# patrickltobing/cyclevae-vc

Measured on AMD Instinct MI355X. Metric: mcep_frames_per_sec_hu1024_ld32_cyc2, higher is better.
Workload: dtype f32 (every matrix product on exact fp32 operands: each operand carried as three fp16 limbs x = l0 + l1/2^11 + l2/2^22, six v_mfma_f32_32x32x16_f16 per product, f32 accumulate; dropped terms < 2^-33 of a product; gates, carried state, projection and outputs f32)

## Files before the change

cyclevae-vc_amd/csrc/cvae_exact3.h:

```cpp
#pragma once
#include <cvae_intrin.h>

#if defined(__HIP_DEVICE_COMPILE__)
#define CVAE_V6_IN_AGPR(x) asm volatile("" : "+a"(x))
#else
#define CVAE_V6_IN_AGPR(x) ((void)0)
#endif

struct Step6Params {
    const float* gx0;
    const float* w2s;
    float* hbuf;
    long mtot;
    float* hx;
    const float* wrec3;
    const float* afold3;
    const float* cfold;
    const float* bhn;
    const float* xt;
    int Tp, Cp;
    int B, Bp, H, T;
    unsigned* flags;
    int* status;
    long long* prof;
    const float* wyT;
    const float* dy;
    int Co;
    int rts;
    int want_f32;
    int exp;
    int backoff;
    const float* gx;
    long gx_bstride;
};

__global__ void k_prep_wrec3(const float* wrec2, float* wrec3, int H, int KPW, int* unfit) {
    const int nch = H >> 4, NB = H >> 3;
    const long idx = (long)blockIdx.x * blockDim.x + threadIdx.x;
    if (idx < (long)NB * 4 * KPW * 512) {
        const int e = (int)(idx & 7), lane = (int)((idx >> 3) & 63);
        const int s = (int)((idx >> 9) % KPW), wave = (int)(((idx >> 9) / KPW) & 3), c = (int)((idx >> 9) / KPW / 4);
        const int col = lane & 31, kh = lane >> 5, g = col >> 3, u = col & 7, j = 8 * c + u;
        const int k = 16 * (wave * KPW + s) + 8 * kh + e;
        float w = 0.0f;
        if (k < H) w = wrec2[((((long)(j >> 4) * 4 + g) * nch + (k >> 4)) * 16 + (j & 15)) * 16 + (k & 15)];
        unsigned short l0, l1, l2;
        cvae_split3_f16(w, l0, l1, l2);
        cvae_flag_unfit(unfit, w);
        unsigned short* dst = (unsigned short*)wrec3 + ((((long)c * 4 + wave) * KPW + s) * 3) * 512 + lane * 8 + e;
        dst[0] = l0;
        dst[512] = l1;
        dst[1024] = l2;
    }
}

__global__ void k_prep_wrec3_l2b(const float* wrec2, unsigned char* w2s, int H, int KPW) {
    const int nch = H >> 4, NB = H >> 3;
    const long idx = (long)blockIdx.x * blockDim.x + threadIdx.x;
    if (idx < (long)NB * 4 * KPW * 512) {
        const int e = (int)(idx & 7), lane = (int)((idx >> 3) & 63);
        const int s = (int)((idx >> 9) % KPW), wave = (int)(((idx >> 9) / KPW) & 3), c = (int)((idx >> 9) / KPW / 4);
        const int col = lane & 31, kh = lane >> 5, g = col >> 3, u = col & 7, j = 8 * c + u;
        const int k = 16 * (wave * KPW + s) + 8 * kh + e;
        float w = 0.0f;
        if (k < H) w = wrec2[((((long)(j >> 4) * 4 + g) * nch + (k >> 4)) * 16 + (j & 15)) * 16 + (k & 15)];
        unsigned short l0, l1;
        unsigned char l2;
        cvae_split3_f16b8(w, l0, l1, l2);
        w2s[idx] = l2;
    }
}

__global__ void k_prep_afold3l(const float* afold, float* afold3, int H, int Kfe, int KFW, int* unfit) {
    const int NB = H >> 3;
    const long idx = (long)blockIdx.x * blockDim.x + threadIdx.x;
    if (idx < (long)NB * 4 * KFW * 512) {
        const int e = (int)(idx & 7), lane = (int)((idx >> 3) & 63);
        const int s = (int)((idx >> 9) % KFW), wave = (int)(((idx >> 9) / KFW) & 3), c = (int)((idx >> 9) / KFW / 4);
        const int col = lane & 31, kh = lane >> 5, g = col >> 3, u = col & 7;
        const int k = 16 * (wave * KFW + s) + 8 * kh + e;
        const float w = (g < 3 && k < Kfe) ? afold[(long)(g * H + 8 * c + u) * Kfe + k] : 0.0f;
        unsigned short l0, l1, l2;
        cvae_split3_f16(w, l0, l1, l2);
        cvae_flag_unfit(unfit, w);
// ... 61 lines not shown
            CVAE_V6_IN_AGPR(w0[s]);
            CVAE_V6_IN_AGPR(w1[s]);
            CVAE_V6_IN_AGPR(w2[s]);
        }
    }
    {
        const float* src = p.afold3 + ((long)c * 4 + wave) * (KFW * 3 * 256);
        float* dst = wfl + wave * (KFW * LIMBS * 256);
#pragma unroll
        for (int s = 0; s < KFW; ++s)
#pragma unroll
            for (int m = 0; m < LIMBS; ++m)
                *(f32x4*)(dst + (s * LIMBS + m) * 256 + lane * 4) = *(const f32x4*)(src + (s * 3 + m) * 256 + lane * 4);
    }
    __syncthreads();
    const float* wfw = wfl + wave * (KFW * LIMBS * 256) + lane * 4;
    const float bhn = p.bhn[j];
    const float cf0 = HOIST ? 0.f : p.cfold[j], cf1 = HOIST ? 0.f : p.cfold[H + j], cf2 = HOIST ? 0.f : p.cfold[2 * H + j];
    const int ntile = ti < nrt ? (nrt - ti + rts - 1) / rts : 0, ntask = p.T * ntile;
    long long pc[PROF ? 4 : 1] = {};
    f32x4 x4[2 * RF];
    f32x2 x2[RF];
    const unsigned char* xw = nullptr;
    auto set_x = [&](int k) {
        const int tt = k / ntile, ii = ti + (k % ntile) * rts;
        xw = (const unsigned char*)p.xt + (((long)ii * p.Tp + tt) * (p.Cp >> 3) + 2 * (wave * KFW) + kh) * 1280;
    };
    auto load_x = [&](int s) {
        x4[2 * (s % RF)] = *(const f32x4*)(xw + s * 2560 + lc * 16);
        x4[2 * (s % RF) + 1] = *(const f32x4*)(xw + s * 2560 + 512 + lc * 16);
        if constexpr (LIMBS == 3) x2[s % RF] = *(const f32x2*)(xw + s * 2560 + 1024 + lc * 8);
    };
    float gq0 = 0.f, gq1 = 0.f, gq2 = 0.f;
    auto load_g = [&](int k) {
        const int tt = k / ntile, gr = (ti + (k % ntile) * rts) * 32 + row;
        if (gr < p.B) {
            const float* g = p.gx + (long)gr * p.gx_bstride + (long)tt * 3 * H + j;
            gq0 = g[0]; gq1 = g[H]; gq2 = g[2 * H];
        }
    };
    constexpr bool FPRE = CVAE_V6_FPRE && !HOIST && LIMBS == 3 && !W2S && KPW <= 16;
    constexpr bool FW0_EARLY = KFW <= 6;
    f32x4 fw[FPRE ? 2 * LIMBS : 1];
    auto load_fw = [&](int s) {
#pragma unroll
        for (int m = 0; m < LIMBS; ++m) fw[(s & 1) * LIMBS + m] = *(const f32x4*)(wfw + (s * LIMBS + m) * 256);
    };
    auto fw_op = [&](int s, int m) -> f32x4 {
        if constexpr (FPRE) return fw[(s & 1) * LIMBS + m];
        else return *(const f32x4*)(wfw + (s * LIMBS + m) * 256);
    };
    float hkeep0 = 0.f, hkeep1 = 0.f;
    const int backoff = (p.exp >> 8) ? (p.exp >> 8) - 1 : p.backoff;
    if constexpr (HOIST) {
        if (ntask > 0) load_g(0);
    } else if (ntask > 0) {
        set_x(0);
#pragma unroll
        for (int s = 0; s < RF; ++s) load_x(s);
    }
    if constexpr (FPRE && FW0_EARLY) { if (ntask > 0) load_fw(0); }
    unsigned fpre = 0u;
    for (int k = 0; k < ntask; ++k) {
        long long c0 = 0;
        if constexpr (PROF) c0 = cvae_clock();
        const int t = k / ntile, i = ti + (k % ntile) * rts;
        const unsigned row0 = (unsigned)(t * p.Bp + i * 32), tile0 = row0 >> 5;
        f32x16 a0 = cvae_zero16(), a1 = cvae_zero16(), a2 = cvae_zero16(), a3 = cvae_zero16();
        if constexpr (FPRE && !FW0_EARLY) load_fw(0);
#pragma unroll
        for (int s = 0; s < KFW; ++s) {
            const f32x4 l0 = x4[2 * (s % RF)], l1 = x4[2 * (s % RF) + 1];
            if constexpr (FPRE) {
                if (s + 1 < KFW) load_fw(s + 1);
                cvae_sched_fence();
            }
            const f32x4 b0 = fw_op(s, 0);
            const f32x4 b1 = fw_op(s, 1);
            a0 = cvae_mfma_32x32x16_f16(l0, b0, a0);
            a1 = cvae_mfma_32x32x16_f16(l0, b1, a1);
            if constexpr (LIMBS == 3) {
                const f32x4 l2 = cvae_bf8x8_to_h8(x2[s % RF]);
                const f32x4 b2 = fw_op(s, 2);
                a2 = cvae_mfma_32x32x16_f16(l1, b1, a2);
                if constexpr (W2S) a2 = cvae_mfma_32x32x16_f16(l0, b2, a2);
                else a3 = cvae_mfma_32x32x16_f16(l0, b2, a3);
                a1 = cvae_mfma_32x32x16_f16(l1, b0, a1);
                a2 = cvae_mfma_32x32x16_f16(l2, b0, a2);
            } else {
                a2 = cvae_mfma_32x32x16_f16(l1, b0, a2);
            }
            cvae_sched_fence();
            if (s + RF < KFW) load_x(s + RF);
        }
        if constexpr (PROF) { const long long c1 = cvae_clock(); pc[0] += c1 - c0; c0 = c1; }
        const bool pre_ok = ntile > 1 && k > 0 && cvae_wave_all(fpre >= (unsigned)t);
        if (t > 0 && !pre_ok) {
            unsigned spins = 0;
            if (ntile == 1)
                for (int q = 0; q < backoff; ++q) cvae_sleep_64();
            for (;;) {
                unsigned f = (unsigned)t;
                if (lane < 2 * KPW && 2 * s_lo + lane < NB) f = cvae_atomic_load_agent(p.flags + (long)i * NB + 2 * s_lo + lane);
                if (cvae_wave_all(f >= (unsigned)t)) break;
                cvae_sleep();
                if (++spins > (1u << 22)) {
                    p.status[0] = 2;
                    break;
                }
            }
        }
        cvae_compiler_fence();
        if constexpr (PROF) { const long long c1 = cvae_clock(); pc[1] += c1 - c0; c0 = c1; }
        const int grow = i * 32 + row;
        const bool live = grow < p.B;
        const bool keep1 = ntile == 2 && (k & 1);
        float gxr = HOIST ? gq0 : cf0, gxz = HOIST ? gq1 : cf1, gxn = HOIST ? gq2 : cf2, hold = keep1 ? hkeep1 : hkeep0;
        auto gate_inputs = [&]() {
            if (live) {
                if (t == 0 && p.gx0) {
                    const float* g0p = p.gx0 + (long)grow * 3 * H + j;
                    gxr += g0p[0]; gxz += g0p[H]; gxn += g0p[2 * H];
                } else if (t == 0 && p.dy) cvae_t0_fix(p.wyT, p.dy, p.Co, H, j, grow, gxr, gxz, gxn);
                if (t == 0) {
                    hold = cvae_buf_load_f1_sc1(hb, (unsigned)(row * 64 + (j & 15) * 4), ((unsigned)(j >> 4) * mtot + row0) * 64u);
                } else if (ntile > 2) {
                    const unsigned so = ((unsigned)(j >> 4) * tstride + tile0) * 2560u, okh = (unsigned)((j >> 3) & 1);
                    const unsigned vo = okh * 512u + (unsigned)(row * 16 + (u >> 1) * 4);
                    const int sh = (u & 1) * 16;
                    const unsigned q0 = __builtin_bit_cast(unsigned, cvae_buf_load_f1_sc1(xb_, vo, so));
                    const unsigned q1 = __builtin_bit_cast(unsigned, cvae_buf_load_f1_sc1(xb_, vo, so + 1024u));
                    float third = 0.0f;
                    if constexpr (LIMBS == 3) {
                        const unsigned q2 = __builtin_bit_cast(unsigned, cvae_buf_load_f1_sc1(xb_, 2048u + okh * 256u + (unsigned)(row * 8 + (u >> 2) * 4), so));
                        third = cvae_bf8_to_f32((unsigned char)(q2 >> ((u & 3) * 8))) * (S1 / CVAE_L2_SCALE);
                    }
                    hold = cvae_f16_bits_to_f32((unsigned short)(q0 >> sh)) + (cvae_f16_bits_to_f32((unsigned short)(q1 >> sh)) + third) * S1;
                }
            }
        };
        if constexpr (KPW >= 32) gate_inputs();
        f32x4 hc[2 * RD];
        f32x2 hb2[RD];
        const unsigned tsel = (p.exp & 1) ? (unsigned)i : tile0;
        auto load_h = [&](int s) {
            const unsigned so = ((unsigned)(s_lo + s) * tstride + tsel) * 2560u;
            hc[2 * (s % RD)] = cvae_buf_load_f4(xb_, voff, so);
            hc[2 * (s % RD) + 1] = cvae_buf_load_f4(xb_, voff, so + 1024u);
            if constexpr (LIMBS == 3) hb2[s % RD] = cvae_buf_load_f2(xb_, voff2, so);
        };
        f32x2 w2r[W2S ? RW : 1];
        const float* w2base = W2S ? p.w2s + ((long)c * 4 + wave) * KPW * 128 + lane * 2 : nullptr;
        auto load_w2 = [&](int s) { w2r[s % RW] = *(const f32x2*)(w2base + s * 128); };
        if constexpr (W2S) {
#pragma unroll
            for (int s = 0; s < RW; ++s) load_w2(s);
        }
#pragma unroll
        for (int s = 0; s < RD; ++s) load_h(s);
        if constexpr (KPW < 32) gate_inputs();
#pragma unroll
        for (int s = 0; s < KPW; ++s) {
            const f32x4 l0 = hc[2 * (s % RD)], l1 = hc[2 * (s % RD) + 1];
// ... 11 lines not shown
            }
            cvae_sched_fence();
            if (s + RD < KPW) load_h(s + RD);
            if constexpr (W2S) { if (s + RW < KPW) load_w2(s + RW); }
        }
        cvae_sched_fence();
        const int xmode = HOIST ? 0 : (p.exp >> 5) & 3;
        if constexpr (HOIST) {
            if (k + 1 < ntask) load_g(k + 1);
        } else {
            if (k + 1 < ntask) set_x(k + 1);
            if (k + 1 < ntask && (xmode == 0 || (xmode == 2 && wave != 0))) {
#pragma unroll
                for (int s = 0; s < RF; ++s) load_x(s);
            }
        }
#pragma unroll
        for (int q = 0; q < 16; ++q)
            red[(wave * 32 + (q & 3) + 8 * (q >> 2) + 4 * kh) * RS + lc] =
                LIMBS == 3 ? a0[q] + (a1[q] + (a2[q] + a3[q]) * S1) * S1 : a0[q] + (a1[q] + a2[q]) * S1;
        if constexpr (PROF) { const long long c1 = cvae_clock(); pc[2] += c1 - c0; c0 = c1; }
        __syncthreads();
        {
            float hn_ = 0.0f;
            if (live) {
                float sg[4];
#pragma unroll
                for (int g = 0; g < 4; ++g)
                    sg[g] = red[(0 * 32 + row) * RS + g * 8 + u] + red[(1 * 32 + row) * RS + g * 8 + u] +
                            red[(2 * 32 + row) * RS + g * 8 + u] + red[(3 * 32 + row) * RS + g * 8 + u];
                const float rg = cvae_sigmoid_fast(gxr + sg[0]);
                const float zg = cvae_sigmoid_fast(gxz + sg[1]);
                const float ng = cvae_tanh_fast(gxn + sg[2] + rg * (sg[3] + bhn));
                hn_ = ng + zg * (hold - ng);
            }
            if (keep1) hkeep1 = hn_; else hkeep0 = hn_;
            hsh[row * 8 + u] = hn_;
            unsigned short l0, l1;
            unsigned char l2;
            cvae_split3_f16b8(hn_, l0, l1, l2);
            hl[row * 8 + u] = l0;
            hl[256 + row * 8 + u] = l1;
            ((unsigned char*)(hl + 512))[row * 8 + u] = l2;
        }
        __syncthreads();
        if (tid < 64) {
            const unsigned so = ((unsigned)(c >> 1) * tstride + tile0 + (unsigned)(p.Bp >> 5)) * 2560u;
            cvae_buf_store_f4_sc1(xb_, (unsigned)(c & 1) * 512u + (unsigned)(tid & 31) * 16u, so + (unsigned)(tid >> 5) * 1024u,
                                  *(const f32x4*)(hl + tid * 8));
            if (LIMBS == 3 && tid < 32)
                cvae_buf_store_f2_sc1(xb_, 2048u + (unsigned)(c & 1) * 256u + (unsigned)tid * 8u, so, *(const f32x2*)(hl + 512 + tid * 4));
            cvae_drain_vmem();
            cvae_wave_barrier();
            if (tid == 0) cvae_atomic_store_agent(p.flags + (long)i * NB + c, (unsigned)(t + 1));
        } else if (tid < 128 && p.want_f32) {
            const int l = tid - 64, r = l >> 1, half = l & 1;
            *(f32x4*)(p.hbuf + (((long)(c >> 1) * p.mtot + row0 + p.Bp + r) * 16 + (c & 1) * 8 + half * 4)) =
                *(const f32x4*)(hsh + r * 8 + half * 4);
        }
        if constexpr (!HOIST) {
            if (k + 1 < ntask && (xmode == 1 || (xmode == 2 && wave == 0))) {
#pragma unroll
                for (int s = 0; s < RF; ++s) load_x(s);
            }
        }
        if (ntile > 1 && k + 1 < ntask) {
            const int kn = k + 1, tn = kn / ntile, in_ = ti + (kn % ntile) * rts;
            fpre = (unsigned)tn;
            if (tn > 0 && lane < 2 * KPW && 2 * s_lo + lane < NB)
                fpre = cvae_atomic_load_agent(p.flags + (long)in_ * NB + 2 * s_lo + lane);
        }
        if constexpr (FPRE && FW0_EARLY) { if (k + 1 < ntask) load_fw(0); }
        if constexpr (PROF) { const long long c1 = cvae_clock(); pc[3] += c1 - c0; c0 = c1; }
    }
    if constexpr (PROF) {
        if (p.prof && tid == 64 * ((p.exp >> 2) & 3))
            for (int q = 0; q < 4; ++q) p.prof[(long)blockIdx.x * 4 + q] = pc[q];
    }
}

struct Out6Params {
    const float* hx;
    long mtot;
    const float* wo3;
    const float* bo2;
    int H, Bp, T, B, ncell, Co, clamp_from;
    float clamp_min;
    float* out[CVAE_MAX_CELLS];
};

__global__ void k_prep_wo3(const float* wo2, float* wo3, int H, int Cop, int NT, int* unfit) {
    const int nk = H >> 4;
    const long idx = (long)blockIdx.x * blockDim.x + threadIdx.x;
    if (idx < (long)NT * nk * 512) {
        const int e = (int)(idx & 7), lane = (int)((idx >> 3) & 63), s = (int)((idx >> 9) % nk), n = (int)((idx >> 9) / nk);
        const int col = 32 * n + (lane & 31), k = 16 * s + 8 * (lane >> 5) + e;
        const float w = col < Cop ? wo2[(long)col * H + k] : 0.0f;
        unsigned short l0, l1, l2;
        cvae_split3_f16(w, l0, l1, l2);
        cvae_flag_unfit(unfit, w);
        unsigned short* dst = (unsigned short*)wo3 + (((long)n * nk + s) * 3) * 512 + lane * 8 + e;
        dst[0] = l0;
        dst[512] = l1;
        dst[1024] = l2;
    }
}

template <int KPW>
__global__ __launch_bounds__(256) void k_outproj_v6(Out6Params p) {
    constexpr float S1 = 1.0f / 2048.0f;
    constexpr int RS = 36;
    const int tid = threadIdx.x, wave = cvae_uniform(tid >> 6), lane = tid & 63, lc = lane & 31, kh = lane >> 5;
    const int nk = p.H >> 4, nt32 = p.Bp >> 5;
    const int n = blockIdx.y;
    const long tile = (long)nt32 + blockIdx.x;
    float* red = (float*)CVAE_SMEM;
    const long tstride = p.mtot >> 5;
    f32x16 a0 = cvae_zero16(), a1 = cvae_zero16(), a2 = cvae_zero16(), a3 = cvae_zero16();
    constexpr int RD = KPW < 4 ? KPW : 4;
    f32x4 ha[2 * RD], wb[3 * RD];
    f32x2 hb[RD];
    auto load = [&](int s) {
        const int sg = wave * KPW + s;
// ... 90 lines not shown
```

cyclevae-vc_amd/csrc/cvae_lib.hip:

```cpp
#include <cvae_intrin.h>

#include <stdarg.h>
#include <stdio.h>
#include <stdlib.h>
#include <string.h>

#include <atomic>
#include <map>
#include <mutex>
#include <new>
#include <utility>
#include <vector>

#include "cvae_kernels.h"
#include "cvae_train_kernels.h"
#include "cvae_deep.h"
#include "cyclevae_hip.h"

namespace {

thread_local char g_err[512] = "";

enum OptId {
    OPT_V6_LIMBS_H64, OPT_NO_LL, OPT_MAX_RT, OPT_LL_BACKOFF, OPT_EXP, OPT_GEMM_FORCE, OPT_GEMM_LOG, OPT_TRAIN_OLD_GEMM,
    OPT_GEMM_TRACE, OPT_TRAIN_PER_STEP, OPT_TRAIN_PROF, OPT_TRAIN_BACKOFF, OPT_TRAIN_FP32_MFMA, OPT_TRAIN_BWD_PER_STEP, OPT_TRAIN_KERNEL, OPT_X3_TILE, OPT_BWD_OVERFLOW_AT, OPT_GEMM_MAX_SPLIT, OPT_BWD_KS, OPT_COOP_LAUNCH, OPT_V6_LIMBS_H2048, OPT_V6_W2S_H64, OPT_STEP_COL_TILES, OPT_TRAIN_PROFILE, OPT_TRAIN_XMAP, OPT_MASKS_ON_SIDE, OPT_V6_BACKOFF, OPT_TRAIN_BWD_BACKOFF, OPT_LL_ROW_PAD, OPT_GEMM_MIN_DEPTH, OPT_TRAIN_BWD_GEOM, OPT_BWD_W3_L1_H64, OPT_TRAIN_FWD_GEOM, OPT_TRAIN_FWD_BACKOFF, OPT_EXACT_RANGE_AT, OPT_DTW_BATCH_COST, OPT_COUNT
};
struct OptEntry { const char* name; long dflt; };
const OptEntry g_opt[OPT_COUNT] = {
    {"v6_limbs_h64", 3},
    {"no_ll", 0},
    {"max_rt", 0},
    {"ll_backoff", -1},
    {"exp", 0},
    {"gemm_force", 0},
    {"gemm_log", 0},
    {"train_old_gemm", 0},
    {"gemm_trace", 0},
    {"train_per_step", 0},
    {"train_prof", 0},
    {"train_backoff", 32},
    {"train_fp32_mfma", 0},
    {"train_bwd_per_step", 0},
    {"train_kernel", 0},
    {"x3_tile", 0},
    {"bwd_overflow_at", 60000},
    {"gemm_max_split", 16},
    {"bwd_ks", 8},
    {"coop_launch", 0},
    {"v6_limbs_h2048", 3},
    {"v6_w2s_h64", 0},
    {"step_col_tiles", 0},
    {"train_profile", 0},
    {"train_xmap", 0},
    {"masks_on_side", 1},
    {"v6_backoff", -1},
    {"train_bwd_backoff", -1},
    {"ll_row_pad", 0},
    {"gemm_min_depth", 128},
    {"train_bwd_geom", -1},
    {"bwd_w3_l1_h64", 0},
    {"train_fwd_geom", -1},
    {"train_fwd_backoff", -1},
    {"exact_range_at", 65504},
    {"dtw_batch_cost", 1},
};

struct ProfEvents {
    std::vector<hipEvent_t> start, stop;
    std::vector<int> rows, cin;
    size_t used = 0;
};
enum { TPROF_FWD = 0, TPROF_BWD = 1, TPROF_GEMM = 2, TPROF_WGRAD = 3, TPROF_CLASSES = 4 };
struct TrainProfEvents {
    std::vector<hipEvent_t> start, stop;
    std::vector<int> cls;
    std::vector<double> flop;
    size_t used = 0;
};
struct SideDone { const void* scratch; hipEvent_t ev; };

}

struct cvae_ctx {
    int32_t* status_sink = nullptr;
    long draw_row0 = 0, draw_rows = 0, draw_frames = 0, draw_parts = 1;
    long opt[OPT_COUNT];
    ProfEvents prof;
    TrainProfEvents tprof;
    hipStream_t side = nullptr;
    SideDone side_done[8] = {};
    hipEvent_t side_ready = nullptr, side_join = nullptr, side_last = nullptr;
    int side_cap = 0;
    hipEvent_t mask_fork = nullptr, mask_join = nullptr;
    unsigned side_evict = 0;
    int32_t* gemm_ran = nullptr;
    std::map<const void*, std::pair<int, unsigned long>> train_var;
    unsigned long train_var_tick = 0;
    std::map<const void*, bool> image_unfit;
    int range_serial = 0;
    std::atomic<unsigned> ll_train_launch{1u};
};

namespace {

thread_local cvae_ctx* tl_ctx = nullptr;
inline cvae_ctx& cx() { return *tl_ctx; }
inline long opt(OptId i) { return tl_ctx->opt[i]; }
struct CtxScope {
    cvae_ctx* prev;
    explicit CtxScope(cvae_ctx* c) : prev(tl_ctx) {
        tl_ctx = c;
        g_cvae_coop_launch = (int)c->opt[OPT_COOP_LAUNCH];
    }
    ~CtxScope() { tl_ctx = prev; }
};

int fail(int code, const char* fmt, ...) {
// ... 129 lines not shown
}
inline bool exact3_fused(const Dims& m) { return find_v6(m) != nullptr; }
inline bool exact3_ok(const Dims& m) { return exact3_fused(m) || find_v6h(m) != nullptr; }
inline int v6_limbs(const Dims& m) {
    return (m.H == 64 && opt(OPT_V6_LIMBS_H64) == 2) || (m.H == 2048 && opt(OPT_V6_LIMBS_H2048) == 2) ? 2 : 3;
}
inline bool v6_w2s(const Dims& m) { return v6_limbs(m) == 3 && (m.H == 2048 || (m.H == 64 && opt(OPT_V6_W2S_H64))); }

struct Prep {
    long afold, afold3, afold_h, afold_t, cfold, wrec, wrec2, wrec_h, wrec_t, wrec_l2b, bhn, wyT, wo, bo, wo2, bo2, wo3, sin_w, sin_b, sout_w,
        sout_b, range, total;
};

Prep prep_layout(const Dims& m, bool sin, bool sout) {
    Prep p;
    long o = 0;
    auto take = [&](long n) { long r = o; o += up(n, 64); return r; };
    p.afold = take((long)m.H3 * m.Kfe);
    p.afold3 = take((long)m.nch * 4 * m.KFW * 3 * 256);
    p.afold_h = take((long)m.nch * 4 * ((m.KFW + 1) / 2) * 6 * 256);
    p.cfold = take(m.H3);
    p.wrec = take((long)(m.H / 4) * m.nch * 256);
    p.wrec2 = take((long)m.nch * 4 * m.nch * 256);
    p.wrec_h = take((long)m.nch * 4 * (m.H / 32) * 2 * 256);
    p.wrec_t = exact3_ok(m) ? take((long)(m.H / 8) * 4 * exact3_kpw(m) * 3 * 256) : -1;
    p.afold_t = exact3_fused(m) ? take((long)(m.H / 8) * 4 * m.KFW * 3 * 256) : -1;
    p.wrec_l2b = exact3_ok(m) ? take((long)(m.H / 8) * 4 * exact3_kpw(m) * 128) : -1;
    p.bhn = take(m.H);
    p.wyT = take((long)m.H3 * m.Co);
    p.wo = take((long)m.Cop * m.H);
    p.bo = take(m.Cop);
    p.wo2 = take((long)m.Cop * m.H);
    p.bo2 = take(m.Cop);
    p.wo3 = exact3_ok(m) ? take((long)((m.Cop + 31) / 32) * (m.H / 16) * 3 * 256) : -1;
    p.sin_w = sin ? take((long)m.C * m.C) : -1;
    p.sin_b = sin ? take(m.C) : -1;
    p.sout_w = sout ? take((long)m.Co * m.Co) : -1;
    p.sout_b = sout ? take(m.Co) : -1;
    p.range = take(64);
    p.total = o;
    return p;
}

struct Work {
    long status, xnp, xs, xs_plane, xt, xt_slack, gx, hbuf, hs, y, dy, gx0, prof, flags, total;
    int Bp, Tp, prof_blocks;
    long mtot;
};

inline int eval_row_pad(const Dims& m, int Brows) {
    return Brows <= 3 ? 16 : (exact3_ok(m) || Brows > 16 ? (int)up(Brows, 32) : 16);
}

Work work_layout(const Dims& m, int Brows, int T) {
    Work w;
    w.Bp = eval_row_pad(m, Brows);
    w.Tp = T + 2 * m.pad;
    w.mtot = (long)(T + 1) * w.Bp;
    long o = 0;
    auto take = [&](long n) { long r = o; o += up(n, 64); return r; };
    w.status = take(64);
    w.xnp = take((long)Brows * w.Tp * m.Cp + 64L * m.KFW + 64);
    w.xs_plane = up((long)Brows * w.Tp * m.Cp + 64L * m.KFW + 64, 8);
    w.xs = take(w.xs_plane);
    w.xt_slack = (64L * m.KFW / 8 + 2) * 640 + 64;
    w.xt = exact3_fused(m) && w.Bp % 32 == 0 ? take(((long)w.Bp * w.Tp * m.Cp * 5 / 2 + w.xt_slack) / 2 + 8) : -1;
    w.gx = take((long)Brows * w.Tp * m.H3);
    w.hbuf = take((long)m.nch * w.mtot * 16);
    w.hs = take((long)m.nch * w.mtot * 24);
    w.y = take((long)T * w.Bp * m.Cop);
    w.dy = take((long)w.Bp * m.Co);
    w.gx0 = take((long)w.Bp * m.H3);
    w.prof_blocks = 256;
    w.prof = take(w.prof_blocks * 8L);
    w.flags = take((long)(w.Bp / 16) * m.nch);
    w.total = o;
    return w;
}

inline int row_tiles_per_block(int cus, int per_tile, int ntiles) {
    int rts = per_tile > 0 ? cus / per_tile : 1;
    rts = rts < 1 ? 1 : (rts > ntiles ? ntiles : rts);
    if (opt(OPT_MAX_RT) >= 1 && opt(OPT_MAX_RT) < rts) rts = (int)opt(OPT_MAX_RT);
    return rts;
}

struct PassFacts {
    bool h_in, y_last, h_last, many_draws;
};
enum { PRO_ROWS = 0, PRO_DRAWS = 1, PRO_TILES = 2 };
enum { PROJ_GEMM = 0, PROJ_FUSED = 1, PROJ_V6 = 2 };
struct EvalPlan {
    int form;
    void (*k6)(Step6Params);
    void (*k5)(Step3Params);
    void (*k4)(Step3Params);
    void (*kout6)(Out6Params);
    int rts;
    int backoff;
    bool limbs;
    bool pairs;
    bool gx0_ready;
    bool want_f32;
    int prologue, proj;
};

inline int plain_projection(const Dims& m, bool y_last) {
    const int ntn = m.Cop / 16;
    return !y_last && (ntn == 1 || ntn == 4 || ntn == 8) ? PROJ_FUSED : PROJ_GEMM;
}

inline bool generic_resident(const Dims& m, int cus) { return cus <= 0 || m.H / 4 <= cus; }

EvalPlan plan_eval_pass(const Dims& m, int Brows, int T, int flags, int cus, bool unfit, const PassFacts& f) {
    EvalPlan pn;
    memset(&pn, 0, sizeof(pn));
    if (unfit) flags &= ~CVAE_FLAG_SPLIT_F16;
    const int Bp = eval_row_pad(m, Brows);
    const long mtot = (long)(T + 1) * Bp;
    const bool persistent = (flags & CVAE_FLAG_PERSISTENT) && T > 1, generic = (flags & CVAE_FLAG_GENERIC_STEP) != 0;
    const bool hoisted = (flags & CVAE_FLAG_HOISTED_FRONTEND) != 0, exact = persistent && (flags & CVAE_FLAG_EXACT3) && !generic;
    const V6Inst* i6 = find_v6(m, v6_limbs(m), v6_w2s(m));
    const V6Inst* i6h = find_v6h(m, v6_limbs(m), v6_w2s(m));
    const Fused16Inst* i16 = find_fused16(m);
    if (exact && Brows <= 3 && T < 65536 && m.H % 64 == 0 && m.H <= 1024 && cus >= m.H / 4 && !opt(OPT_NO_LL)) {
        pn.form = CVAE_EVAL_LL;
        pn.backoff = opt(OPT_LL_BACKOFF) >= 0 ? (int)opt(OPT_LL_BACKOFF) : (Brows == 1 ? 22 : 20);
    } else if (exact && !unfit && !hoisted && i6 && Bp % 32 == 0 && cus >= m.H / 8 && (long)m.nch * mtot * 80 < (1L << 31)) {
        pn.form = CVAE_EVAL_V6;
        pn.k6 = (flags & CVAE_FLAG_STEP_TIMING) && i6->fn_prof ? i6->fn_prof : i6->fn;
        pn.rts = row_tiles_per_block(cus, m.H / 8, Bp / 32);
        pn.backoff = opt(OPT_V6_BACKOFF) >= 0 ? (int)opt(OPT_V6_BACKOFF) : (m.H == 1024 ? (m.KFW > 6 ? 10 : (m.KFW == 6 ? 16 : 8)) : 0);
    } else if (exact && !unfit && !hoisted && i6h && Bp % 32 == 0 && cus >= m.H / 8 && (long)m.nch * mtot * 80 < (1L << 31)) {
        pn.form = CVAE_EVAL_V6H;
        i6 = i6h;
        pn.k6 = (flags & CVAE_FLAG_STEP_TIMING) && i6h->fn_prof ? i6h->fn_prof : i6h->fn;
        pn.rts = row_tiles_per_block(cus, m.H / 8, Bp / 32);
        pn.backoff = opt(OPT_V6_BACKOFF) >= 0 ? (int)opt(OPT_V6_BACKOFF) : 0;
    } else if (persistent && !generic && (m.H == 1024 || m.H == 64) && cus >= m.nch && (long)m.nch * mtot * 64 < (1L << 31)) {
        pn.form = hoisted || !i16 ? CVAE_EVAL_V2 : ((flags & CVAE_FLAG_SPLIT_F16) ? CVAE_EVAL_V5 : CVAE_EVAL_V4);
        if (i16) pn.k5 = i16->v5, pn.k4 = i16->v4;
        pn.rts = row_tiles_per_block(cus, m.nch, Bp / 16);
    } else {
        pn.form = persistent && generic_resident(m, cus) ? CVAE_EVAL_GENERIC : CVAE_EVAL_PER_STEP;
    }
    const bool v6f = pn.form == CVAE_EVAL_V6, v6 = v6f || pn.form == CVAE_EVAL_V6H;
    pn.limbs = v6 || pn.form == CVAE_EVAL_V5;
    pn.pairs = !v6 && (flags & CVAE_FLAG_SPLIT_F16);
    pn.gx0_ready = v6 && !f.h_in;
    pn.want_f32 = v6 && (i6->limbs != 3 || f.y_last || f.h_last || (opt(OPT_EXP) & 16));
    pn.prologue = v6f ? PRO_TILES : (f.many_draws ? PRO_DRAWS : PRO_ROWS);
    if (!f.y_last && v6 && i6->limbs == 3) {
        pn.proj = PROJ_V6;
        for (const Out6Inst& o : g_out6_inst)
            if (o.H == m.H) pn.kout6 = o.fn;
    } else {
        pn.proj = plain_projection(m, f.y_last);
    }
    return pn;
}

bool prof_begin(hipStream_t st, int rows = 0, int cin = 0) {
    if (cx().prof.used == cx().prof.start.size()) {
        hipEvent_t a, b;
        if (hipEventCreate(&a) != hipSuccess || hipEventCreate(&b) != hipSuccess) return false;
        cx().prof.start.push_back(a);
        cx().prof.stop.push_back(b);
        cx().prof.rows.push_back(0);
        cx().prof.cin.push_back(0);
    }
    cx().prof.rows[cx().prof.used] = rows;
    cx().prof.cin[cx().prof.used] = cin;
    return hipEventRecord(cx().prof.start[cx().prof.used], st) == hipSuccess;
}
void prof_end(hipStream_t st) {
    (void)hipEventRecord(cx().prof.stop[cx().prof.used], st);
    cx().prof.used++;
}

struct TrainProf {
    hipStream_t st;
    bool on;
    TrainProf(hipStream_t st_, int cls, double flop) : st(st_), on(false) {
        if (!opt(OPT_TRAIN_PROFILE)) return;
        if (cx().tprof.used == cx().tprof.start.size()) {
            hipEvent_t a, b;
            if (hipEventCreate(&a) != hipSuccess || hipEventCreate(&b) != hipSuccess) return;
            cx().tprof.start.push_back(a); cx().tprof.stop.push_back(b); cx().tprof.cls.push_back(0); cx().tprof.flop.push_back(0.0);
        }
        cx().tprof.cls[cx().tprof.used] = cls;
        cx().tprof.flop[cx().tprof.used] = flop;
        on = hipEventRecord(cx().tprof.start[cx().tprof.used], st) == hipSuccess;
    }
    void end() {
        if (!on) return;
        (void)hipEventRecord(cx().tprof.stop[cx().tprof.used], st);
        cx().tprof.used++;
        on = false;
    }
// ... 181 lines not shown
    hipLaunchKernelGGL((k_gemm_nt<2, 4, 4, 1, true>), dim3(nblk(N, 64), nblk(M, 128)), dim3(256), 0, st, hbuf + (long)Bp * 16, 0L, mtot,
                       P + pl.wo, (long)m.H, P + pl.bo, y, (long)m.Cop, M, N, m.H);
    for (int c = 0; c < ncell; ++c) {
        EpiParams ep;
        ep.y = y; ep.ldy = m.Cop;
        ep.sout_w = d->has_scale_out ? P + pl.sout_w : nullptr;
        ep.sout_b = d->has_scale_out ? P + pl.sout_b : nullptr;
        ep.clamp_from = d->has_scale_out ? -1 : clamp_dim(clamp_lat_dim);
        ep.clamp_min = clamp_floor(clamp_lat_dim);
        ep.B = B; ep.Bp = Bp; ep.T = T; ep.Co = m.Co; ep.b0 = c * B;
        ep.trj_out = cells[c].trj_out; ep.y_last = cells[c].y_last;
        ep.t_last = last_slot(cells[c].in, T) - 1;
        hipLaunchKernelGGL((k_epilogue), dim3(B * T), dim3(64), m.Co * sizeof(float), st, ep);
    }
}

void run_last_states(const Dims& m, const PassRows& r, const float* hbuf, hipStream_t st) {
    for (int c = 0; c < r.ncell; ++c)
        if (r.cells[c].h_last)
            hipLaunchKernelGGL((k_hlast), dim3(nblk((long)r.B * m.H, 256)), dim3(256), 0, st, hbuf, r.mtot, r.cells[c].h_last, r.B, r.Bp,
                               m.H, last_slot(r.cells[c].in, r.T), c * r.B);
}

int run_pass(const Dims& m, const cvae_net_desc* d, const float* P, const Cell* cells, int ncell, int B, int T,
             int clamp_lat_dim, float* ws, int* status, int flags, hipStream_t st, bool clear_status = false) {
    const Prep pl = prep_layout(m, d->has_scale_in != 0, d->has_scale_out != 0);
    const int Brows = ncell * B;
    const Work wl = work_layout(m, Brows, T);
    int* const ws_status = status;
    if (cx().status_sink) status = cx().status_sink;
    const PassRows rows = {cells, ncell, B, T, wl.Bp, wl.mtot};
    if (int rc = check_cells(m, rows)) return rc;
    unsigned* bar = (unsigned*)(ws + wl.status) + 8;
    float* xnp = ws + wl.xnp;
    float* gx = ws + wl.gx;
    float* hbuf = ws + wl.hbuf;
    float* dy = ws + wl.dy;
    unsigned* hflags = (unsigned*)(ws + wl.flags);
    long long* const step_prof = (flags & CVAE_FLAG_STEP_TIMING) ? (long long*)(ws + wl.prof) : nullptr;
    const int cus = cu_count();
    PassFacts facts = {};
    for (int c = 0; c < ncell; ++c) {
        facts.h_in = facts.h_in || cells[c].h_in != nullptr;
        facts.y_last = facts.y_last || cells[c].y_last != nullptr;
        facts.h_last = facts.h_last || cells[c].h_last != nullptr;
        facts.many_draws = facts.many_draws || (cells[c].in->lat && cells[c].in->n_draws > 1);
    }
    const EvalPlan pn = plan_eval_pass(m, Brows, T, flags, cus, image_known_unfit(P), facts);

    {
        ProTargets o = {};
        o.shape = pn.prologue; o.xnp = xnp; o.dy = dy;
        o.slot0 = hbuf;
        o.zero_words = hflags; o.nzero = wl.Bp / 16 * m.nch;
        o.zero_status = clear_status ? status : nullptr;
        o.zero_status_n = cx().status_sink ? 4 : 8;
        o.ws_status = ws_status; o.limbs = pn.limbs; o.new_call = clear_status;
        const bool triples = pn.form == CVAE_EVAL_V6 || pn.form == CVAE_EVAL_V6H;
        o.hx = triples ? ws + wl.hs : nullptr;
        o.xt = pn.form == CVAE_EVAL_V6 ? ws + wl.xt : nullptr;
        o.nxt_slack = (int)wl.xt_slack;
        o.hs = pn.pairs ? ws + wl.hs : nullptr;
        o.xs = pn.pairs ? ws + wl.xs : nullptr;
        o.xs_plane = wl.xs_plane;
        o.gx0 = pn.gx0_ready ? ws + wl.gx0 : nullptr;
        o.ll_counter = pn.form == CVAE_EVAL_LL ? (unsigned*)(ws + wl.status) + 16 : nullptr;
        run_prologue(m, d, P, pl, rows, o, st);
    }

    const size_t lds2 = (4 * 16 * 84 + 16 * 16) * sizeof(float);
    const bool prof = (flags & CVAE_FLAG_PROFILE) && prof_begin(st, ncell * B, m.C);
    const auto refused = [](hipError_t e) {
        if (e == hipSuccess) return false;
        (void)hipGetLastError();
        return true;
    };
    int form = pn.form;
    if (form == CVAE_EVAL_LL || form == CVAE_EVAL_V6H || form <= CVAE_EVAL_V2) run_front_end_gemm(m, P, pl, xnp, gx, Brows, wl.Tp, st);
    switch (form) {
    case CVAE_EVAL_LL: {
        StepLLParams q;
        q.hbuf = hbuf; q.mtot = wl.mtot; q.xbuf = ws + wl.hs; q.wrec2 = P + pl.wrec2; q.gx = gx; q.gx_bstride = (long)wl.Tp * m.H3;
        q.bhn = P + pl.bhn; q.B = Brows; q.Bp = wl.Bp; q.H = m.H; q.T = T; q.status = status;
        q.prof = step_prof;
        q.wyT = P + pl.wyT; q.dy = dy; q.Co = m.Co;
        q.dbg = (int*)(ws + wl.status);
        q.backoff = pn.backoff;
        q.nonce_src = (const unsigned*)(ws + wl.status) + 16;
        const dim3 gl(m.H / 4);
        const size_t ldsl = (size_t)(2 * 64 * 49 + 4 * 48) * sizeof(float);
        const hipError_t e = cvae_launch_coop(Brows == 1 ? k_gru_steps_ll<1> : Brows == 2 ? k_gru_steps_ll<2> : k_gru_steps_ll<3>, gl,
                                              dim3(256), ldsl, st, q);
        if (refused(e)) return fail(-3, "small-batch recurrent kernel failed to launch: %s", hipGetErrorString(e));
        break;
    }
    case CVAE_EVAL_V6:
    case CVAE_EVAL_V6H: {
        const bool fused = form == CVAE_EVAL_V6;
        Step6Params q;
        q.hbuf = hbuf; q.mtot = wl.mtot; q.hx = ws + wl.hs; q.wrec3 = P + pl.wrec_t; q.afold3 = fused ? P + pl.afold_t : nullptr; q.w2s = P + pl.wrec_l2b;
        q.cfold = P + pl.cfold; q.bhn = P + pl.bhn; q.xt = fused ? ws + wl.xt : nullptr; q.Tp = wl.Tp; q.Cp = m.Cp;
        q.gx = fused ? nullptr : gx; q.gx_bstride = (long)wl.Tp * m.H3;
        q.B = Brows; q.Bp = wl.Bp; q.H = m.H; q.T = T; q.flags = hflags; q.status = status;
        q.prof = step_prof;
        q.wyT = P + pl.wyT; q.dy = dy; q.Co = m.Co;
        q.gx0 = pn.gx0_ready ? ws + wl.gx0 : nullptr;
        q.want_f32 = pn.want_f32 ? 1 : 0;
        q.rts = pn.rts;
        q.exp = (int)opt(OPT_EXP);
        q.backoff = pn.backoff;
        const size_t lds6 = (size_t)(4 * 32 * 40 + 32 * 8 + 384 + (fused ? 4 * m.KFW * v6_limbs(m) * 256 : 0)) * sizeof(float);
        const hipError_t e = cvae_launch_coop(pn.k6, dim3(m.H / 8 * pn.rts), dim3(256), lds6, st, q);
        if (refused(e)) return fail(-3, "exact-operand recurrent kernel failed to launch: %s", hipGetErrorString(e));
        break;
    }
    case CVAE_EVAL_V5:
    case CVAE_EVAL_V4: {
        Step3Params q;
        q.hbuf = hbuf; q.mtot = wl.mtot; q.wrec2 = P + pl.wrec2; q.cfold = P + pl.cfold;
        q.xnp = xnp; q.Tp = wl.Tp; q.Cp = m.Cp; q.bhn = P + pl.bhn; q.B = Brows; q.Bp = wl.Bp; q.H = m.H; q.T = T;
        q.flags = hflags; q.status = status;
        q.prof = step_prof;
        q.wyT = P + pl.wyT; q.dy = dy; q.Co = m.Co;
        q.rts = pn.rts;
        q.hs = ws + wl.hs; q.wrec_h = P + pl.wrec_h; q.xs = ws + wl.xs; q.xs_plane = wl.xs_plane;
        q.exp = (int)opt(OPT_EXP);
        const dim3 g(m.nch * pn.rts);
        if (form == CVAE_EVAL_V5) {
            q.afold2 = P + pl.afold_h;
            const size_t lds5 = lds2 + (size_t)4 * ((m.KFW + 1) / 2) * 6 * 256 * sizeof(float);
            if (!refused(cvae_launch_coop(pn.k5, g, dim3(256), lds5, st, q))) break;
        }
        q.afold2 = P + pl.afold3;
        const size_t lds4 = lds2 + (size_t)4 * m.KFW * 3 * 256 * sizeof(float);
        if (!refused(cvae_launch_coop(pn.k4, g, dim3(256), lds4, st, q))) break;
        run_front_end_gemm(m, P, pl, xnp, gx, Brows, wl.Tp, st);
        form = CVAE_EVAL_V2;
    }
        [[fallthrough]];
    case CVAE_EVAL_V2: {
        Step2Params q;
        q.hbuf = hbuf; q.mtot = wl.mtot; q.wrec2 = P + pl.wrec2; q.gx = gx; q.gx_bstride = (long)wl.Tp * m.H3;
        q.bhn = P + pl.bhn; q.B = Brows; q.Bp = wl.Bp; q.H = m.H; q.T = T; q.flags = hflags; q.status = status;
        q.prof = step_prof;
        q.wyT = P + pl.wyT; q.dy = dy; q.Co = m.Co;
        if (!refused(cvae_launch_coop(m.H == 1024 ? k_gru_steps_v2<16> : k_gru_steps_v2<1>, dim3(m.nch, pn.rts), dim3(256), lds2, st, q))) break;
        form = generic_resident(m, cus) ? CVAE_EVAL_GENERIC : CVAE_EVAL_PER_STEP;
    }
        [[fallthrough]];
    default: {
        const size_t step_lds = 4 * 64 * 20 * sizeof(float);
        StepParams sp;
        sp.hbuf = hbuf; sp.mtot = wl.mtot; sp.wrec = P + pl.wrec; sp.gx = gx; sp.gx_bstride = (long)wl.Tp * m.H3;
        sp.bhn = P + pl.bhn; sp.B = Brows; sp.Bp = wl.Bp; sp.H = m.H; sp.T = T; sp.t0 = 0; sp.bar = bar; sp.status = status;
        sp.nwg = (unsigned)(m.H / 4);
        sp.prof = nullptr;
        sp.wyT = P + pl.wyT; sp.dy = dy; sp.Co = m.Co;
        if (form == CVAE_EVAL_GENERIC) {
            CVAE_HIP_OK(hipMemsetAsync(bar, 0, 8 * sizeof(unsigned), st));
            if (!refused(cvae_launch_coop(k_gru_steps<true>, dim3(sp.nwg), dim3(256), step_lds, st, sp))) break;
        }
        for (int t = 0; t < T; ++t) {
            sp.t0 = t;
// ... 578 lines not shown
```

Measured before the change: 1.327 million.

## Replicate per-step ready flags per XCD and add optional adaptive spin backoff

Each block now publishes its step-completion flag into 8 padded copies, and readers poll the copy selected by blockIdx mod 8, which follows the round-robin XCD placement. The goal is to keep the spinning atomic loads local to each XCD instead of contending on one shared flag line across dies. The default backoff is retuned lower when copies are on, and an opt-in adaptive backoff adjusts the pre-spin sleep from observed spins. The cost is extra flag stores per step and a larger flag region to zero.

```diff
diff --git a/cyclevae-vc_amd/csrc/cvae_exact3.h b/cyclevae-vc_amd/csrc/cvae_exact3.h
--- a/cyclevae-vc_amd/csrc/cvae_exact3.h
+++ b/cyclevae-vc_amd/csrc/cvae_exact3.h
@@ -21,6 +21,7 @@
     int Tp, Cp;
     int B, Bp, H, T;
     unsigned* flags;
+    int fcopies;
     int* status;
     long long* prof;
     const float* wyT;
@@ -30,6 +31,7 @@
     int want_f32;
     int exp;
     int backoff;
+    int adapt;
     const float* gx;
     long gx_bstride;
 };
@@ -197,6 +199,11 @@
     };
     float hkeep0 = 0.f, hkeep1 = 0.f;
     const int backoff = (p.exp >> 8) ? (p.exp >> 8) - 1 : p.backoff;
+    const bool adapt = p.adapt && !(p.exp >> 8);
+    int delay = backoff;
+    const int fcopies = p.fcopies, fpad = fcopies > 1 ? (NB + 31) & ~31 : NB;
+    const long ftile = (long)fcopies * fpad;
+    const unsigned* frd = p.flags + ((int)blockIdx.x & (fcopies - 1)) * fpad;
     if constexpr (HOIST) {
         if (ntask > 0) load_g(0);
     } else if (ntask > 0) {
@@ -243,10 +250,10 @@
         if (t > 0 && !pre_ok) {
             unsigned spins = 0;
             if (ntile == 1)
-                for (int q = 0; q < backoff; ++q) cvae_sleep_64();
+                for (int q = 0; q < delay; ++q) cvae_sleep_64();
             for (;;) {
                 unsigned f = (unsigned)t;
-                if (lane < 2 * KPW && 2 * s_lo + lane < NB) f = cvae_atomic_load_agent(p.flags + (long)i * NB + 2 * s_lo + lane);
+                if (lane < 2 * KPW && 2 * s_lo + lane < NB) f = cvae_atomic_load_agent(frd + (long)i * ftile + 2 * s_lo + lane);
                 if (cvae_wave_all(f >= (unsigned)t)) break;
                 cvae_sleep();
                 if (++spins > (1u << 22)) {
@@ -254,6 +261,7 @@
                     break;
                 }
             }
+            if (adapt && ntile == 1) delay = spins == 0 ? (delay > 0 ? delay - 1 : 0) : (delay < 2 * backoff ? delay + 1 : 2 * backoff);
         }
         cvae_compiler_fence();
         if constexpr (PROF) { const long long c1 = cvae_clock(); pc[1] += c1 - c0; c0 = c1; }
@@ -371,7 +379,7 @@
                 cvae_buf_store_f2_sc1(xb_, 2048u + (unsigned)(c & 1) * 256u + (unsigned)tid * 8u, so, *(const f32x2*)(hl + 512 + tid * 4));
             cvae_drain_vmem();
             cvae_wave_barrier();
-            if (tid == 0) cvae_atomic_store_agent(p.flags + (long)i * NB + c, (unsigned)(t + 1));
+            if (tid < fcopies) cvae_atomic_store_agent(p.flags + (long)i * ftile + tid * fpad + c, (unsigned)(t + 1));
         } else if (tid < 128 && p.want_f32) {
             const int l = tid - 64, r = l >> 1, half = l & 1;
             *(f32x4*)(p.hbuf + (((long)(c >> 1) * p.mtot + row0 + p.Bp + r) * 16 + (c & 1) * 8 + half * 4)) =
@@ -387,7 +395,7 @@
             const int kn = k + 1, tn = kn / ntile, in_ = ti + (kn % ntile) * rts;
             fpre = (unsigned)tn;
             if (tn > 0 && lane < 2 * KPW && 2 * s_lo + lane < NB)
-                fpre = cvae_atomic_load_agent(p.flags + (long)in_ * NB + 2 * s_lo + lane);
+                fpre = cvae_atomic_load_agent(frd + (long)in_ * ftile + 2 * s_lo + lane);
         }
         if constexpr (FPRE && FW0_EARLY) { if (k + 1 < ntask) load_fw(0); }
         if constexpr (PROF) { const long long c1 = cvae_clock(); pc[3] += c1 - c0; c0 = c1; }
diff --git a/cyclevae-vc_amd/csrc/cvae_lib.hip b/cyclevae-vc_amd/csrc/cvae_lib.hip
--- a/cyclevae-vc_amd/csrc/cvae_lib.hip
+++ b/cyclevae-vc_amd/csrc/cvae_lib.hip
@@ -23,7 +23,7 @@
 
 enum OptId {
     OPT_V6_LIMBS_H64, OPT_NO_LL, OPT_MAX_RT, OPT_LL_BACKOFF, OPT_EXP, OPT_GEMM_FORCE, OPT_GEMM_LOG, OPT_TRAIN_OLD_GEMM,
-    OPT_GEMM_TRACE, OPT_TRAIN_PER_STEP, OPT_TRAIN_PROF, OPT_TRAIN_BACKOFF, OPT_TRAIN_FP32_MFMA, OPT_TRAIN_BWD_PER_STEP, OPT_TRAIN_KERNEL, OPT_X3_TILE, OPT_BWD_OVERFLOW_AT, OPT_GEMM_MAX_SPLIT, OPT_BWD_KS, OPT_COOP_LAUNCH, OPT_V6_LIMBS_H2048, OPT_V6_W2S_H64, OPT_STEP_COL_TILES, OPT_TRAIN_PROFILE, OPT_TRAIN_XMAP, OPT_MASKS_ON_SIDE, OPT_V6_BACKOFF, OPT_TRAIN_BWD_BACKOFF, OPT_LL_ROW_PAD, OPT_GEMM_MIN_DEPTH, OPT_TRAIN_BWD_GEOM, OPT_BWD_W3_L1_H64, OPT_TRAIN_FWD_GEOM, OPT_TRAIN_FWD_BACKOFF, OPT_EXACT_RANGE_AT, OPT_DTW_BATCH_COST, OPT_COUNT
+    OPT_GEMM_TRACE, OPT_TRAIN_PER_STEP, OPT_TRAIN_PROF, OPT_TRAIN_BACKOFF, OPT_TRAIN_FP32_MFMA, OPT_TRAIN_BWD_PER_STEP, OPT_TRAIN_KERNEL, OPT_X3_TILE, OPT_BWD_OVERFLOW_AT, OPT_GEMM_MAX_SPLIT, OPT_BWD_KS, OPT_COOP_LAUNCH, OPT_V6_LIMBS_H2048, OPT_V6_W2S_H64, OPT_STEP_COL_TILES, OPT_TRAIN_PROFILE, OPT_TRAIN_XMAP, OPT_MASKS_ON_SIDE, OPT_V6_BACKOFF, OPT_TRAIN_BWD_BACKOFF, OPT_LL_ROW_PAD, OPT_GEMM_MIN_DEPTH, OPT_TRAIN_BWD_GEOM, OPT_BWD_W3_L1_H64, OPT_TRAIN_FWD_GEOM, OPT_TRAIN_FWD_BACKOFF, OPT_EXACT_RANGE_AT, OPT_DTW_BATCH_COST, OPT_V6_FLAG_COPIES, OPT_V6_BACKOFF_ADAPT, OPT_COUNT
 };
 struct OptEntry { const char* name; long dflt; };
 const OptEntry g_opt[OPT_COUNT] = {
@@ -63,6 +63,8 @@
     {"train_fwd_backoff", -1},
     {"exact_range_at", 65504},
     {"dtw_batch_cost", 1},
+    {"v6_flag_copies", 8},
+    {"v6_backoff_adapt", 0},
 };
 
 struct ProfEvents {
@@ -298,6 +300,11 @@
     return Brows <= 3 ? 16 : (exact3_ok(m) || Brows > 16 ? (int)up(Brows, 32) : 16);
 }
 
+constexpr int V6_FLAG_COPIES_MAX = 8;
+inline long v6_flag_words(const Dims& m, int Bp, int copies) {
+    return (long)(Bp / 32) * (copies > 1 ? copies * up(m.H / 8, 32) : m.H / 8);
+}
+
 Work work_layout(const Dims& m, int Brows, int T) {
     Work w;
     w.Bp = eval_row_pad(m, Brows);
@@ -319,7 +326,8 @@
     w.gx0 = take((long)w.Bp * m.H3);
     w.prof_blocks = 256;
     w.prof = take(w.prof_blocks * 8L);
-    w.flags = take((long)(w.Bp / 16) * m.nch);
+    const long f16 = (long)(w.Bp / 16) * m.nch, f6 = v6_flag_words(m, w.Bp, V6_FLAG_COPIES_MAX);
+    w.flags = take(f16 > f6 ? f16 : f6);
     w.total = o;
     return w;
 }
@@ -344,6 +352,8 @@
     void (*kout6)(Out6Params);
     int rts;
     int backoff;
+    int fcopies;
+    bool adapt;
     bool limbs;
     bool pairs;
     bool gx0_ready;
@@ -376,7 +386,9 @@
         pn.form = CVAE_EVAL_V6;
         pn.k6 = (flags & CVAE_FLAG_STEP_TIMING) && i6->fn_prof ? i6->fn_prof : i6->fn;
         pn.rts = row_tiles_per_block(cus, m.H / 8, Bp / 32);
-        pn.backoff = opt(OPT_V6_BACKOFF) >= 0 ? (int)opt(OPT_V6_BACKOFF) : (m.H == 1024 ? (m.KFW > 6 ? 10 : (m.KFW == 6 ? 16 : 8)) : 0);
+        const bool per_xcd = opt(OPT_V6_FLAG_COPIES) == V6_FLAG_COPIES_MAX;
+        const int swept = per_xcd ? (m.KFW > 6 ? 6 : (m.KFW == 6 ? 10 : 8)) : (m.KFW > 6 ? 10 : (m.KFW == 6 ? 16 : 8));
+        pn.backoff = opt(OPT_V6_BACKOFF) >= 0 ? (int)opt(OPT_V6_BACKOFF) : (m.H == 1024 ? swept : 0);
     } else if (exact && !unfit && !hoisted && i6h && Bp % 32 == 0 && cus >= m.H / 8 && (long)m.nch * mtot * 80 < (1L << 31)) {
         pn.form = CVAE_EVAL_V6H;
         i6 = i6h;
@@ -391,6 +403,8 @@
         pn.form = persistent && generic_resident(m, cus) ? CVAE_EVAL_GENERIC : CVAE_EVAL_PER_STEP;
     }
     const bool v6f = pn.form == CVAE_EVAL_V6, v6 = v6f || pn.form == CVAE_EVAL_V6H;
+    pn.fcopies = v6 && opt(OPT_V6_FLAG_COPIES) == V6_FLAG_COPIES_MAX ? V6_FLAG_COPIES_MAX : 1;
+    pn.adapt = v6 && pn.backoff > 0 && (opt(OPT_V6_BACKOFF_ADAPT) == 2 || (opt(OPT_V6_BACKOFF_ADAPT) == 1 && opt(OPT_V6_BACKOFF) < 0));
     pn.limbs = v6 || pn.form == CVAE_EVAL_V5;
     pn.pairs = !v6 && (flags & CVAE_FLAG_SPLIT_F16);
     pn.gx0_ready = v6 && !f.h_in;
@@ -678,7 +692,8 @@
         ProTargets o = {};
         o.shape = pn.prologue; o.xnp = xnp; o.dy = dy;
         o.slot0 = hbuf;
-        o.zero_words = hflags; o.nzero = wl.Bp / 16 * m.nch;
+        o.zero_words = hflags;
+        o.nzero = pn.form == CVAE_EVAL_V6 || pn.form == CVAE_EVAL_V6H ? (int)v6_flag_words(m, wl.Bp, pn.fcopies) : wl.Bp / 16 * m.nch;
         o.zero_status = clear_status ? status : nullptr;
         o.zero_status_n = cx().status_sink ? 4 : 8;
         o.ws_status = ws_status; o.limbs = pn.limbs; o.new_call = clear_status;
@@ -735,6 +750,7 @@
         q.rts = pn.rts;
         q.exp = (int)opt(OPT_EXP);
         q.backoff = pn.backoff;
+        q.fcopies = pn.fcopies; q.adapt = pn.adapt ? 1 : 0;
         const size_t lds6 = (size_t)(4 * 32 * 40 + 32 * 8 + 384 + (fused ? 4 * m.KFW * v6_limbs(m) * 256 : 0)) * sizeof(float);
         const hipError_t e = cvae_launch_coop(pn.k6, dim3(m.H / 8 * pn.rts), dim3(256), lds6, st, q);
         if (refused(e)) return fail(-3, "exact-operand recurrent kernel failed to launch: %s", hipGetErrorString(e));
```

After: 1.340 million (median of 6 runs). About the same (+0.9%).
